# peterWon/D-LIOM

Hardware: NVIDIA H100
Metric: scans/sec (64-beam, 10 Hz) per GPU; pose RMSE vs reference CPU (higher is better)
Workload: dtype f32 (indices, scores) + f64 (pre-integration, least squares)

## Files before the change

d-liom_b200/csrc/dl_voxel.cu:

```cuda
#include <algorithm>
#include <cstdlib>

#include "dl_internal.cuh"

namespace dl {
namespace {

constexpr uint32_t kEmpty = 0xFFFFFFFFu;
constexpr int kBlock = 256;

__device__ __forceinline__ uint32_t hash_cell(const Int3& c) {
  uint32_t h = (uint32_t)c.x * 73856093u ^ (uint32_t)c.y * 19349663u ^ (uint32_t)c.z * 83492791u;
  h ^= h >> 15;
  h *= 0x2c1b3c6du;
  h ^= h >> 12;
  return h;
}
__device__ __forceinline__ Int3 row_cell(const float* __restrict__ pts, int stride, uint32_t row, float res) {
  const float* p = pts + (size_t)row * stride;
  return cell_index(Vec3f{p[0], p[1], p[2]}, res);
}

template <typename RowOf>
__device__ __forceinline__ uint32_t table_insert(uint32_t* table, uint32_t mask, const float* pts, int stride,
// ... 16 lines not shown
                                                              float res, uint32_t* table, int64_t table_cap,
                                                              uint32_t* slot) {
  const int b = blockIdx.y;
  const int n = counts[b];
  const float* pts = points + (size_t)b * cap * stride;
  uint32_t* tab = table + (size_t)b * table_cap;
  const uint32_t mask = (uint32_t)table_cap - 1;
  for (int i = blockIdx.x * kBlock + threadIdx.x; i < n; i += gridDim.x * kBlock) {
    const Int3 c = row_cell(pts, stride, i, res);
    slot[(size_t)b * cap + i] = table_insert(tab, mask, pts, stride, res, c, (uint32_t)i, [](uint32_t id) { return id; });
  }
}

__device__ __forceinline__ int block_exclusive_scan(int value, int* total) {
  __shared__ int warp_sums[kBlock / 32];
  const int lane = threadIdx.x & 31, warp = threadIdx.x >> 5;
  int inc = value;
#pragma unroll
  for (int d = 1; d < 32; d <<= 1) {
    const int o = __shfl_up_sync(0xffffffffu, inc, d);
    if (lane >= d) inc += o;
  }
  __syncthreads();
  if (lane == 31) warp_sums[warp] = inc;
  __syncthreads();
  int base = 0, sum = 0;
#pragma unroll
  for (int w = 0; w < kBlock / 32; ++w) {
    const int s = warp_sums[w];
    if (w < warp) base += s;
    sum += s;
  }
  *total = sum;
  return base + inc - value;
}

__global__ void __launch_bounds__(kBlock) voxel_count_kernel(const int32_t* __restrict__ counts, int64_t cap,
                                                             const uint32_t* __restrict__ table, int64_t table_cap,
                                                             const uint32_t* __restrict__ slot, int32_t* block_counts,
                                                             int tiles) {
  const int b = blockIdx.y;
  const int n = counts[b];
  const int i = blockIdx.x * kBlock + threadIdx.x;
  int flag = 0;
  if (i < n) flag = __ldcg(table + (size_t)b * table_cap + slot[(size_t)b * cap + i]) == (uint32_t)i;
  int total;
  block_exclusive_scan(flag, &total);
  if (threadIdx.x == 0) block_counts[(size_t)b * tiles + blockIdx.x] = total;
}

__global__ void __launch_bounds__(kBlock) voxel_scatter_kernel(const int32_t* __restrict__ counts, int64_t cap,
                                                               const uint32_t* __restrict__ table, int64_t table_cap,
                                                               const uint32_t* __restrict__ slot,
                                                               const int32_t* __restrict__ block_counts, int tiles,
                                                               int32_t* keep, int32_t* keep_counts) {
  const int b = blockIdx.y;
  const int n = counts[b];
  __shared__ int tile_base;
  int partial = 0;
  for (int t = threadIdx.x; t < (int)blockIdx.x; t += kBlock) partial += block_counts[(size_t)b * tiles + t];
  int total;
  block_exclusive_scan(partial, &total);
  if (threadIdx.x == 0) tile_base = total;
  __syncthreads();
  const int i = blockIdx.x * kBlock + threadIdx.x;
  int flag = 0;
  if (i < n) flag = __ldcg(table + (size_t)b * table_cap + slot[(size_t)b * cap + i]) == (uint32_t)i;
  const int off = block_exclusive_scan(flag, &total);
  if (flag) keep[(size_t)b * cap + tile_base + off] = i;
  if (blockIdx.x == gridDim.x - 1 && threadIdx.x == 0) keep_counts[b] = tile_base + total;
}

__global__ void voxel_indices_kernel(const float* __restrict__ points, int stride, int64_t n, float res,
                                     int32_t* __restrict__ out) {
  const int64_t i = (int64_t)blockIdx.x * blockDim.x + threadIdx.x;
  if (i >= n) return;
  const float* p = points + (size_t)i * stride;
  const Int3 c = cell_index(Vec3f{p[0], p[1], p[2]}, make_divider(res));
  out[3 * i] = c.x;
  out[3 * i + 1] = c.y;
  out[3 * i + 2] = c.z;
}

constexpr int kAdaptiveBlock = 1024;
constexpr int kAdaptiveWarps = kAdaptiveBlock / 32;

__device__ __forceinline__ int block_sum_1024(int v) {
  __shared__ int ws[32];
  __shared__ int result;
  const int lane = threadIdx.x & 31, warp = threadIdx.x >> 5;
#pragma unroll
  for (int d = 16; d > 0; d >>= 1) v += __shfl_xor_sync(0xffffffffu, v, d);
  __syncthreads();
  if (lane == 0) ws[warp] = v;
  __syncthreads();
  if (warp == 0) {
    int s = lane < kAdaptiveWarps ? ws[lane] : 0;
#pragma unroll
    for (int d = 16; d > 0; d >>= 1) s += __shfl_xor_sync(0xffffffffu, s, d);
    if (lane == 0) result = s;
  }
  __syncthreads();
  return result;
}

__device__ __forceinline__ int warp_bases_1024(int warp_value, int* total) {
  __shared__ int ws[kAdaptiveWarps], wb[kAdaptiveWarps + 1];
  const int lane = threadIdx.x & 31, warp = threadIdx.x >> 5;
  __syncthreads();
  if (lane == 0) ws[warp] = warp_value;
  __syncthreads();
  if (warp == 0) {
    const int v = ws[lane];
    int inc = v;
#pragma unroll
    for (int d = 1; d < 32; d <<= 1) {
      const int o = __shfl_up_sync(0xffffffffu, inc, d);
      if (lane >= d) inc += o;
    }
    wb[lane] = inc - v;
    if (lane == 31) wb[kAdaptiveWarps] = inc;
  }
  __syncthreads();
  *total = wb[kAdaptiveWarps];
  return wb[warp];
}

template <typename Pred, typename Emit>
__device__ __forceinline__ int block_compact_1024(int n, Pred pred, Emit emit) {
  const int lane = threadIdx.x & 31, warp = threadIdx.x >> 5;
  const int chunk = ((n + kAdaptiveBlock - 1) / kAdaptiveBlock) * 32;
  const int begin = warp * chunk, end = min(n, begin + chunk);
  int count = 0;
  for (int base = begin; base < end; base += 128) {
    bool f[4];
#pragma unroll
    for (int u = 0; u < 4; ++u) {
      const int i = base + 32 * u + lane;
      f[u] = i < end && pred(i);
    }
#pragma unroll
    for (int u = 0; u < 4; ++u) count += __popc(__ballot_sync(0xffffffffu, f[u]));
  }
  int total;
  int pos = warp_bases_1024(count, &total);
  for (int base = begin; base < end; base += 128) {
    bool f[4];
#pragma unroll
    for (int u = 0; u < 4; ++u) {
      const int i = base + 32 * u + lane;
      f[u] = i < end && pred(i);
    }
#pragma unroll
    for (int u = 0; u < 4; ++u) {
      const unsigned ballot = __ballot_sync(0xffffffffu, f[u]);
      if (f[u]) emit(pos + __popc(ballot & ((1u << lane) - 1)), base + 32 * u + lane);
      pos += __popc(ballot);
    }
  }
  __syncthreads();
  return total;
}

template <typename RunPass>
__device__ __forceinline__ bool adaptive_search(const AdaptiveParams& opt, RunPass run_pass, float* result_edge) {
  *result_edge = opt.max_length;
  int result_count = run_pass(opt.max_length);
  if (result_count < 0) return false;
  if ((float)result_count >= opt.min_num_points) return true;
  for (float high_length = opt.max_length; high_length > 1e-2f * opt.max_length; high_length /= 2.f) {
    float low_length = high_length / 2.f;
    result_count = run_pass(low_length);
    if (result_count < 0) return false;
    *result_edge = low_length;
    if ((float)result_count >= opt.min_num_points) {
      while ((high_length - low_length) / low_length > 1e-1f) {
        const float mid_length = (low_length + high_length) / 2.f;
        const int candidate = run_pass(mid_length);
        if (candidate < 0) return false;
        if ((float)candidate >= opt.min_num_points) {
          low_length = mid_length;
          *result_edge = mid_length;
        } else {
          high_length = mid_length;
        }
      }
      return true;
    }
  }
  return true;
}

constexpr int kFastPoints = 8;
constexpr int kFastSlots = 4096;
constexpr int kFastExtra = 14336;
constexpr int kFastCapacity = kFastPoints * 1024 + kFastExtra;
static_assert(kFastCapacity / 1024 <= 32, "the compaction keeps one round count per lane");
constexpr unsigned long long kEmptyKey = 0xFFFFFFFFFFFFFFFFull;

struct FastTable {
  unsigned long long keys[kFastSlots];
  uint32_t mins[kFastSlots];
  float extra[kFastExtra * 3];
};

__device__ __forceinline__ bool pack_cell(const Int3& c, unsigned long long* key) {
  const int lim = 1 << 20;
  if (c.x < -lim || c.x >= lim - 1 || c.y < -lim || c.y >= lim - 1 || c.z < -lim || c.z >= lim - 1) return false;
  *key = ((unsigned long long)(c.x + lim) << 42) | ((unsigned long long)(c.y + lim) << 21) | (unsigned long long)(c.z + lim);
  return true;
}
__device__ __forceinline__ uint32_t hash_key(unsigned long long k) {
  k ^= k >> 33;
  k *= 0xff51afd7ed558ccdull;
  k ^= k >> 29;
  return (uint32_t)k;
}

__device__ __forceinline__ int fast_insert(FastTable& tab, bool have, float x, float y, float z, int j,
                                           const CellDivider& edge, int* fail_flag) {
  const int lane = threadIdx.x & 31;
  unsigned long long key = kEmptyKey - 1 - lane;
  bool ok = true;
  if (have) ok = pack_cell(cell_index(Vec3f{x, y, z}, edge), &key);
  if (!ok) *fail_flag = 1;
  const unsigned peers = __match_any_sync(0xffffffffu, key);
  int claimed = 0;
  if (have && ok && (__ffs(peers) - 1) == lane) {
    uint32_t h = hash_key(key) & (kFastSlots - 1);
    int probes = 0;
    for (;;) {
      const unsigned long long prev = atomicCAS(&tab.keys[h], kEmptyKey, key);
      if (prev == kEmptyKey) claimed = 1;
      if (prev == kEmptyKey || prev == key) {
        atomicMin(&tab.mins[h], (uint32_t)j);
        break;
      }
      h = (h + 1) & (kFastSlots - 1);
      if (++probes >= kFastSlots) {
        *fail_flag = 1;
        break;
      }
    }
  }
  return claimed;
}

__device__ __forceinline__ int fast_pass(FastTable& tab, const float (&px)[kFastPoints], const float (&py)[kFastPoints],
                                         const float (&pz)[kFastPoints], int m, float edge_length, int* fail_flag) {
  const CellDivider edge = make_divider(edge_length);
  for (int i = threadIdx.x; i < kFastSlots; i += kAdaptiveBlock) {
    tab.keys[i] = kEmptyKey;
    tab.mins[i] = 0xFFFFFFFFu;
  }
  __syncthreads();
  int claims = 0;
#pragma unroll
  for (int k = 0; k < kFastPoints; ++k) {
    if (k * kAdaptiveBlock >= m) break;
    const int j = k * kAdaptiveBlock + threadIdx.x;
    claims += fast_insert(tab, j < m, px[k], py[k], pz[k], j, edge, fail_flag);
  }
  for (int base = kFastPoints * kAdaptiveBlock; base < m; base += kAdaptiveBlock) {
    const int j = base + threadIdx.x;
    const float* e = tab.extra + (size_t)(j - kFastPoints * kAdaptiveBlock) * 3;
    const bool have = j < m;
    claims += fast_insert(tab, have, have ? e[0] : 0.f, have ? e[1] : 0.f, have ? e[2] : 0.f, j, edge, fail_flag);
  }
  const int total = block_sum_1024(claims);
  return *fail_flag ? -1 : total;
}

constexpr int kByteCells = (int)((sizeof(unsigned long long) + sizeof(uint32_t)) * kFastSlots);
struct CloudBox {
  float lo[3], hi[3];
};
__device__ __forceinline__ int byte_map_pass(FastTable& tab, const CloudBox& box, const float (&px)[kFastPoints],
                                             const float (&py)[kFastPoints], const float (&pz)[kFastPoints], int m, float edge_length,
                                             int* fail_flag) {
  const CellDivider edge = make_divider(edge_length);
  const Int3 lo = cell_index(Vec3f{box.lo[0], box.lo[1], box.lo[2]}, edge), hi = cell_index(Vec3f{box.hi[0], box.hi[1], box.hi[2]}, edge);
  const long long nx = (long long)hi.x - lo.x + 1, ny = (long long)hi.y - lo.y + 1, nz = (long long)hi.z - lo.z + 1;
  if (nx <= 0 || ny <= 0 || nz <= 0 || nx > kByteCells || ny > kByteCells || nz > kByteCells || nx * ny * nz > kByteCells) return -2;
  const int inx = (int)nx, iny = (int)ny, cells = (int)(nx * ny * nz);
  uint8_t* map = reinterpret_cast<uint8_t*>(&tab);
  uint4* map4 = reinterpret_cast<uint4*>(&tab);
  const int words16 = (cells + 15) >> 4;
  for (int i = threadIdx.x; i < words16; i += kAdaptiveBlock) map4[i] = make_uint4(0u, 0u, 0u, 0u);
  __syncthreads();
  auto mark = [&](float x, float y, float z) {
    const Int3 c = cell_index(Vec3f{x, y, z}, edge);
    const unsigned idx = (unsigned)(((c.z - lo.z) * iny + (c.y - lo.y)) * inx + (c.x - lo.x));
    if (idx < (unsigned)cells) map[idx] = 1;
    else *fail_flag = 1;
  };
#pragma unroll
  for (int k = 0; k < kFastPoints; ++k) {
    if (k * kAdaptiveBlock >= m) break;
    if (k * kAdaptiveBlock + (int)threadIdx.x < m) mark(px[k], py[k], pz[k]);
  }
  for (int j = kFastPoints * kAdaptiveBlock + threadIdx.x; j < m; j += kAdaptiveBlock) {
    const float* e = tab.extra + (size_t)(j - kFastPoints * kAdaptiveBlock) * 3;
    mark(e[0], e[1], e[2]);
  }
  __syncthreads();
  int local = 0;
  for (int i = threadIdx.x; i < words16; i += kAdaptiveBlock) {
    const uint4 v = map4[i];
    local += __popc(v.x) + __popc(v.y) + __popc(v.z) + __popc(v.w);
  }
  const int total = block_sum_1024(local);
  return *fail_flag ? -1 : total;
}

__device__ __forceinline__ bool fast_survives(const FastTable& tab, float x, float y, float z, float edge, int j) {
  unsigned long long key;
  pack_cell(cell_index(Vec3f{x, y, z}, make_divider(edge)), &key);
  uint32_t h = hash_key(key) & (kFastSlots - 1);
  while (tab.keys[h] != key) h = (h + 1) & (kFastSlots - 1);
  return tab.mins[h] == (uint32_t)j;
}

__global__ void __launch_bounds__(kAdaptiveBlock) adaptive_voxel_kernel(
    const float* __restrict__ points, int stride, int64_t cap, const int32_t* __restrict__ counts,
    const AdaptiveParams* __restrict__ filters, int num_filters, uint32_t* table, int64_t table_cap,
    uint32_t* scratch , int32_t* keep, int32_t* keep_counts,
    float* passes, int32_t* num_passes, int32_t* cropped_counts, const int32_t* __restrict__ need) {
  extern __shared__ __align__(16) unsigned char smem_raw[];
  FastTable& fast = *reinterpret_cast<FastTable*>(smem_raw);
  __shared__ int fail_flag;
  const int pair = blockIdx.x;
  if (need && need[4 * pair] == 0) return;
  const int b = pair / num_filters;
  const AdaptiveParams opt = filters[pair % num_filters];
  const int n = counts[b];
  const float* pts = points + (size_t)b * cap * stride;
  uint32_t* tab = table + (size_t)pair * table_cap;
  uint32_t* rows = scratch + (size_t)pair * 2 * cap;
  uint32_t* slot = rows + cap;
  int32_t* out = keep + (size_t)pair * cap;
  float* pass_log = passes + (size_t)pair * 32;
  int npass = 0;
  if (threadIdx.x == 0) fail_flag = 0;

  const int m = block_compact_1024(
      n,
      [&](int i) {
        const float* p = pts + (size_t)i * stride;
        return norm3(Vec3f{p[0], p[1], p[2]}) <= opt.max_range;
      },
      [&](int pos, int i) { rows[pos] = (uint32_t)i; });
  if (threadIdx.x == 0 && cropped_counts) cropped_counts[pair] = m;

  if ((float)m <= opt.min_num_points) {
    for (int j = threadIdx.x; j < m; j += kAdaptiveBlock) out[j] = (int32_t)rows[j];
    if (threadIdx.x == 0) {
      keep_counts[pair] = m;
      num_passes[pair] = 0;
    }
    return;
  }
  auto log_pass = [&](float edge) {
    if (threadIdx.x == 0 && npass < 32) pass_log[npass] = edge;
    ++npass;
  };

  if (m <= kFastCapacity) {
    float px[kFastPoints], py[kFastPoints], pz[kFastPoints];
#pragma unroll
    for (int k = 0; k < kFastPoints; ++k) {
      const int j = k * kAdaptiveBlock + threadIdx.x;
      px[k] = py[k] = pz[k] = 0.f;
      if (j < m) {
        const float* p = pts + (size_t)rows[j] * stride;
        px[k] = p[0]; py[k] = p[1]; pz[k] = p[2];
      }
    }
    for (int j = kFastPoints * kAdaptiveBlock + threadIdx.x; j < m; j += kAdaptiveBlock) {
      const float* p = pts + (size_t)rows[j] * stride;
      float* e = fast.extra + (size_t)(j - kFastPoints * kAdaptiveBlock) * 3;
      e[0] = p[0]; e[1] = p[1]; e[2] = p[2];
    }
    __shared__ CloudBox box;
    __shared__ float box_warp[6][kAdaptiveWarps];
    {
      float lo3[3] = {3.4e38f, 3.4e38f, 3.4e38f}, hi3[3] = {-3.4e38f, -3.4e38f, -3.4e38f};
      auto grow = [&](float x, float y, float z) {
        lo3[0] = fminf(lo3[0], x); lo3[1] = fminf(lo3[1], y); lo3[2] = fminf(lo3[2], z);
        hi3[0] = fmaxf(hi3[0], x); hi3[1] = fmaxf(hi3[1], y); hi3[2] = fmaxf(hi3[2], z);
      };
#pragma unroll
      for (int k = 0; k < kFastPoints; ++k)
        if (k * kAdaptiveBlock + (int)threadIdx.x < m) grow(px[k], py[k], pz[k]);
      for (int j = kFastPoints * kAdaptiveBlock + threadIdx.x; j < m; j += kAdaptiveBlock) {
        const float* p = pts + (size_t)rows[j] * stride;
        grow(p[0], p[1], p[2]);
      }
#pragma unroll
      for (int a3 = 0; a3 < 3; ++a3)
#pragma unroll
        for (int d = 16; d > 0; d >>= 1) {
          lo3[a3] = fminf(lo3[a3], __shfl_xor_sync(0xffffffffu, lo3[a3], d));
          hi3[a3] = fmaxf(hi3[a3], __shfl_xor_sync(0xffffffffu, hi3[a3], d));
        }
      const int lane = threadIdx.x & 31, warp = threadIdx.x >> 5;
      if (lane == 0)
#pragma unroll
        for (int a3 = 0; a3 < 3; ++a3) {
          box_warp[a3][warp] = lo3[a3];
          box_warp[3 + a3][warp] = hi3[a3];
        }
      __syncthreads();
      if (threadIdx.x < 6) {
        float v = box_warp[threadIdx.x][0];
        for (int w = 1; w < kAdaptiveWarps; ++w) v = threadIdx.x < 3 ? fminf(v, box_warp[threadIdx.x][w]) : fmaxf(v, box_warp[threadIdx.x][w]);
        if (threadIdx.x < 3) box.lo[threadIdx.x] = v; else box.hi[threadIdx.x - 3] = v;
      }
    }
    __syncthreads();
    float last_edge = -1.f, result_edge = 0.f;
    const bool ok = adaptive_search(
        opt,
        [&](float edge) {
          log_pass(edge);
          const int count = byte_map_pass(fast, box, px, py, pz, m, edge, &fail_flag);
          if (count != -2) {
            last_edge = -1.f;
            return count;
          }
          last_edge = edge;
          return fast_pass(fast, px, py, pz, m, edge, &fail_flag);
        },
        &result_edge);
    bool done = ok;
    if (ok && last_edge != result_edge) done = fast_pass(fast, px, py, pz, m, result_edge, &fail_flag) >= 0;
    if (done) {
      __shared__ int seq[32 * kAdaptiveWarps];
      const int lane = threadIdx.x & 31, warp = threadIdx.x >> 5;
      const int rounds = (m + kAdaptiveBlock - 1) / kAdaptiveBlock;
      uint32_t flags = 0;
      int my_round_count = 0;
      auto test_round = [&](int k, float x, float y, float z) {
        const int j = k * kAdaptiveBlock + threadIdx.x;
        const bool f = j < m && fast_survives(fast, x, y, z, result_edge, j);
        const unsigned ballot = __ballot_sync(0xffffffffu, f);
        if (f) flags |= 1u << k;
        if (lane == k) my_round_count = __popc(ballot);
      };
#pragma unroll
      for (int k = 0; k < kFastPoints; ++k) {
        if (k >= rounds) break;
        test_round(k, px[k], py[k], pz[k]);
      }
      for (int k = kFastPoints; k < rounds; ++k) {
        const float* e = fast.extra + (size_t)(min(k * kAdaptiveBlock + (int)threadIdx.x, m - 1) - kFastPoints * kAdaptiveBlock) * 3;
        test_round(k, e[0], e[1], e[2]);
      }
      if (lane < rounds) seq[lane * kAdaptiveWarps + warp] = my_round_count;
      __syncthreads();
      const int entries = rounds * kAdaptiveWarps;
      const int v = (int)threadIdx.x < entries ? seq[threadIdx.x] : 0;
      int inc = v;
#pragma unroll
      for (int d = 1; d < 32; d <<= 1) {
        const int o = __shfl_up_sync(0xffffffffu, inc, d);
        if (lane >= d) inc += o;
      }
      int kept;
      const int wbase = warp_bases_1024(__shfl_sync(0xffffffffu, inc, 31), &kept);
      if ((int)threadIdx.x < entries) seq[threadIdx.x] = wbase + inc - v;
      __syncthreads();
      for (int k = 0; k < rounds; ++k) {
        const bool f = (flags >> k) & 1u;
        const unsigned ballot = __ballot_sync(0xffffffffu, f);
        if (f) out[seq[k * kAdaptiveWarps + warp] + __popc(ballot & ((1u << lane) - 1))] = (int32_t)rows[k * kAdaptiveBlock + threadIdx.x];
      }
      if (threadIdx.x == 0) {
        keep_counts[pair] = kept;
        num_passes[pair] = npass;
      }
      return;
    }
    npass = 0;
    __syncthreads();
  }

  uint32_t eff_cap = 64;
  while (eff_cap < 2u * (uint32_t)m) eff_cap <<= 1;
  if (eff_cap > (uint32_t)table_cap) eff_cap = (uint32_t)table_cap;
  const uint32_t mask = eff_cap - 1;
  float last_edge = -1.f;
  auto run_pass = [&](float edge) -> int {
    for (uint32_t i = threadIdx.x; i < eff_cap; i += kAdaptiveBlock) tab[i] = kEmpty;
    __syncthreads();
    for (int j = threadIdx.x; j < m; j += kAdaptiveBlock) {
      const Int3 c = row_cell(pts, stride, rows[j], edge);
      slot[j] = table_insert(tab, mask, pts, stride, edge, c, (uint32_t)j, [&](uint32_t id) { return rows[id]; });
    }
    __syncthreads();
    int local = 0;
    for (int j = threadIdx.x; j < m; j += kAdaptiveBlock) local += __ldcg(tab + slot[j]) == (uint32_t)j;
    last_edge = edge;
    return block_sum_1024(local);
  };
  float result_edge = 0.f;
  adaptive_search(
      opt,
      [&](float edge) {
        log_pass(edge);
        return run_pass(edge);
      },
      &result_edge);
  if (last_edge != result_edge) run_pass(result_edge);
  const int kept = block_compact_1024(
      m, [&](int j) { return __ldcg(tab + slot[j]) == (uint32_t)j; }, [&](int pos, int j) { out[pos] = (int32_t)rows[j]; });
  if (threadIdx.x == 0) {
    keep_counts[pair] = kept;
    num_passes[pair] = npass;
  }
}

constexpr int kEdgeSlots = 8192;
struct EdgeMeta {
  int32_t cropped, voxels, fail, need;
};
__device__ __forceinline__ unsigned long long* edge_keys(uint32_t* table, int64_t table_cap, int pair) {
  return reinterpret_cast<unsigned long long*>(table + (size_t)pair * table_cap);
}
__device__ __forceinline__ uint32_t* edge_mins(uint32_t* table, int64_t table_cap, int pair) {
  return table + (size_t)pair * table_cap + 2 * kEdgeSlots;
}

__global__ void __launch_bounds__(kBlock) adaptive_first_insert_kernel(const float* __restrict__ points, int stride, int64_t cap,
                                                                       const int32_t* __restrict__ counts,
                                                                       const AdaptiveParams* __restrict__ filters, int num_filters,
                                                                       uint32_t* table, int64_t table_cap, uint8_t* win, EdgeMeta* meta) {
  const int pair = blockIdx.y, b = pair / num_filters;
  const AdaptiveParams opt = filters[pair % num_filters];
  const int n = counts[b];
  const float* pts = points + (size_t)b * cap * stride;
  unsigned long long* keys = edge_keys(table, table_cap, pair);
  uint32_t* mins = edge_mins(table, table_cap, pair);
  uint8_t* w = win + (size_t)pair * cap;
  const CellDivider edge = make_divider(opt.max_length);
  int cropped = 0;
  for (int base = blockIdx.x * kBlock; base < n; base += gridDim.x * kBlock) {
    const int i = base + threadIdx.x;
    bool in = false;
    Vec3f p{0.f, 0.f, 0.f};
    if (i < n) {
      const float* q = pts + (size_t)i * stride;
      p = {q[0], q[1], q[2]};
      in = norm3(p) <= opt.max_range;
      w[i] = in ? 2 : 0;
    }
    cropped += in;
    if (in) {
      unsigned long long key;
      if (!pack_cell(cell_index(p, edge), &key)) {
        meta[pair].fail = 1;
      } else {
        uint32_t h = hash_key(key) & (kEdgeSlots - 1);
        int probes = 0;
        for (;;) {
          const unsigned long long prev = atomicCAS(keys + h, kEmptyKey, key);
          if (prev == kEmptyKey || prev == key) {
            atomicMin(mins + h, (uint32_t)i);
            break;
          }
          h = (h + 1) & (kEdgeSlots - 1);
          if (++probes >= kEdgeSlots) {
            meta[pair].fail = 1;
            break;
          }
        }
      }
    }
  }
#pragma unroll
  for (int d = 16; d > 0; d >>= 1) cropped += __shfl_xor_sync(0xffffffffu, cropped, d);
  if ((threadIdx.x & 31) == 0 && cropped) atomicAdd(&meta[pair].cropped, cropped);
}

__global__ void __launch_bounds__(kBlock) adaptive_first_mark_kernel(uint32_t* table, int64_t table_cap, int64_t cap, uint8_t* win,
                                                                     EdgeMeta* meta) {
  const int pair = blockIdx.y;
  const uint32_t* mins = edge_mins(table, table_cap, pair);
  const int h = blockIdx.x * kBlock + threadIdx.x;
  const uint32_t m = __ldcg(mins + h);
  const bool used = m != kEmpty;
  if (used) win[(size_t)pair * cap + m] = 3;
  const int c = __syncthreads_count(used);
  if (threadIdx.x == 0 && c) atomicAdd(&meta[pair].voxels, c);
}

__device__ __forceinline__ int edge_mode(const EdgeMeta& m, const AdaptiveParams& opt) {
  if (m.fail) return 0;
// ... 76 lines not shown

}

int launch_voxel_filter(dl_context* ctx, const float* points, int stride, int64_t cap, const int32_t* counts, int batch,
                        float resolution, uint32_t* table, int64_t table_cap, uint32_t* slot, int32_t* keep,
                        int32_t* keep_counts, int32_t* block_counts) {
  if (batch <= 0 || cap <= 0) return DL_OK;
  DL_CUDA(ctx, cudaMemsetAsync(table, 0xFF, (size_t)batch * table_cap * sizeof(uint32_t), ctx->stream));
  const int tiles = (int)((cap + kBlock - 1) / kBlock);
  const dim3 grid(tiles, batch);
  voxel_insert_kernel<<<grid, kBlock, 0, ctx->stream>>>(points, stride, cap, counts, resolution, table, table_cap, slot);
  DL_LAUNCH_CHECK(ctx, "voxel_insert_kernel");
  voxel_count_kernel<<<grid, kBlock, 0, ctx->stream>>>(counts, cap, table, table_cap, slot, block_counts, tiles);
  DL_LAUNCH_CHECK(ctx, "voxel_count_kernel");
  voxel_scatter_kernel<<<grid, kBlock, 0, ctx->stream>>>(counts, cap, table, table_cap, slot, block_counts, tiles, keep,
                                                         keep_counts);
  DL_LAUNCH_CHECK(ctx, "voxel_scatter_kernel");
  return DL_OK;
}

int launch_voxel_indices(dl_context* ctx, const float* points, int stride, int64_t n, float resolution, int32_t* out) {
  if (n <= 0) return DL_OK;
  voxel_indices_kernel<<<(unsigned)((n + 255) / 256), 256, 0, ctx->stream>>>(points, stride, n, resolution, out);
  DL_LAUNCH_CHECK(ctx, "voxel_indices_kernel");
  return DL_OK;
}

size_t adaptive_first_pass_bytes(int pairs, int64_t cap) {
  const size_t tiles = (size_t)((cap + kBlock - 1) / kBlock);
  return (((size_t)pairs * cap + 255) & ~size_t(255)) + (size_t)pairs * tiles * 4 + (size_t)pairs * sizeof(EdgeMeta) + 256;
}

int launch_adaptive_voxel_filter(dl_context* ctx, const float* points, int stride, int64_t cap, const int32_t* counts,
                                 int batch, const AdaptiveParams* filters_dev, int num_filters, uint32_t* table,
                                 int64_t table_cap, uint32_t* scratch, int32_t* keep, int32_t* keep_counts,
                                 float* passes, int32_t* num_passes, int32_t* cropped_counts, void* first_pass_scratch) {
  if (batch <= 0 || num_filters <= 0) return DL_OK;
  const int pairs = batch * num_filters;
  const int tiles = (int)((cap + kBlock - 1) / kBlock);
  bool first_pass = first_pass_scratch && (size_t)table_cap * 4 >= (size_t)kEdgeSlots * 12;
  if (first_pass && !ctx->h_adaptive_stats) {
    if (cudaMallocHost((void**)&ctx->h_adaptive_stats, 2 * sizeof(int32_t)) != cudaSuccess ||
        cudaMalloc((void**)&ctx->d_adaptive_stats, 2 * sizeof(int32_t)) != cudaSuccess) {
      cudaGetLastError();
      ctx->h_adaptive_stats = nullptr;
    } else {
      ctx->h_adaptive_stats[0] = ctx->h_adaptive_stats[1] = 0;
    }
  }
  int32_t* stats = nullptr;
  if (first_pass && ctx->h_adaptive_stats) {
    const int32_t fell = ctx->h_adaptive_stats[0], probed = ctx->h_adaptive_stats[1];
    const bool probe = (ctx->adaptive_calls++ % 16) == 0;
    if (!probe && probed > 0 && 2 * fell > probed) first_pass = false;
    if (first_pass && probe) stats = ctx->d_adaptive_stats;
  }
  const int32_t* need = nullptr;
  if (first_pass) {
    uint8_t* win = reinterpret_cast<uint8_t*>(first_pass_scratch);
    int32_t* tile_counts = reinterpret_cast<int32_t*>(win + (((size_t)pairs * cap + 255) & ~size_t(255)));
    EdgeMeta* meta = reinterpret_cast<EdgeMeta*>(tile_counts + (size_t)pairs * tiles);
    DL_CUDA(ctx, cudaMemset2DAsync(table, (size_t)table_cap * 4, 0xFF, (size_t)kEdgeSlots * 12, (size_t)pairs, ctx->stream));
    DL_CUDA(ctx, cudaMemsetAsync(meta, 0, sizeof(EdgeMeta) * pairs, ctx->stream));
    if (stats) DL_CUDA(ctx, cudaMemsetAsync(stats, 0, 2 * sizeof(int32_t), ctx->stream));
    const int insert_tiles = std::min(tiles, 96);
    adaptive_first_insert_kernel<<<dim3(insert_tiles, pairs), kBlock, 0, ctx->stream>>>(points, stride, cap, counts, filters_dev,
                                                                                         num_filters, table, table_cap, win, meta);
    DL_LAUNCH_CHECK(ctx, "adaptive_first_insert_kernel");
    adaptive_first_mark_kernel<<<dim3(kEdgeSlots / kBlock, pairs), kBlock, 0, ctx->stream>>>(table, table_cap, cap, win, meta);
    DL_LAUNCH_CHECK(ctx, "adaptive_first_mark_kernel");
    adaptive_first_count_kernel<<<dim3(tiles, pairs), kBlock, 0, ctx->stream>>>(counts, filters_dev, num_filters, cap, win, meta,
                                                                                 tile_counts, tiles);
    DL_LAUNCH_CHECK(ctx, "adaptive_first_count_kernel");
    adaptive_first_prefix_kernel<<<pairs, kBlock, 0, ctx->stream>>>(counts, filters_dev, num_filters, meta, tile_counts, tiles,
                                                                    keep_counts, passes, num_passes, cropped_counts, stats);
    DL_LAUNCH_CHECK(ctx, "adaptive_first_prefix_kernel");
    if (stats)
      DL_CUDA(ctx, cudaMemcpyAsync(ctx->h_adaptive_stats, stats, 2 * sizeof(int32_t), cudaMemcpyDeviceToHost, ctx->stream));
    adaptive_first_scatter_kernel<<<dim3(tiles, pairs), kBlock, 0, ctx->stream>>>(counts, filters_dev, num_filters, cap, win, meta,
                                                                                   tile_counts, tiles, keep);
    DL_LAUNCH_CHECK(ctx, "adaptive_first_scatter_kernel");
    need = &meta->need;
  }
  DL_CUDA(ctx, cudaFuncSetAttribute(adaptive_voxel_kernel, cudaFuncAttributeMaxDynamicSharedMemorySize, (int)sizeof(FastTable)));
  adaptive_voxel_kernel<<<pairs, kAdaptiveBlock, sizeof(FastTable), ctx->stream>>>(
      points, stride, cap, counts, filters_dev, num_filters, table, table_cap, scratch, keep, keep_counts, passes,
      num_passes, cropped_counts, need);
  DL_LAUNCH_CHECK(ctx, "adaptive_voxel_kernel");
  return DL_OK;
}

}
```

Baseline: 110,100.

## Restructure adaptive voxel search into multi-edge count sweeps with speculative edges

Rewrites the adaptive voxel kernel: instead of caching points in registers/shared memory and running one hash or byte-map pass per candidate edge, it replays the search against a table of known counts. It evaluates up to three speculative edges per sweep over global points using packed occupancy bitmaps in a 32KB static shared union. The final survivors go through a small shared hash, and output order comes from a rank sort. The block shrinks from 1024 to 512 threads with two blocks per SM, and a fast rounding-based cell index is added with an exact fallback. It risks more global reads per sweep, a quadratic rank sort when many voxels survive, and falling back to the global-table path when more than 2048 cells survive or the bounding box overflows the map.

```diff
diff --git a/d-liom_b200/csrc/dl_voxel.cu b/d-liom_b200/csrc/dl_voxel.cu
--- a/d-liom_b200/csrc/dl_voxel.cu
+++ b/d-liom_b200/csrc/dl_voxel.cu
@@ -122,11 +122,16 @@
   out[3 * i + 2] = c.z;
 }
 
-constexpr int kAdaptiveBlock = 1024;
-constexpr int kAdaptiveWarps = kAdaptiveBlock / 32;
-
-__device__ __forceinline__ int block_sum_1024(int v) {
-  __shared__ int ws[32];
+constexpr int kSearchBlock = 512;
+constexpr int kSearchWarps = kSearchBlock / 32;
+constexpr int kMapBytes = 32768;
+constexpr int kResultSlots = 2048;
+constexpr int kMaxAhead = 3;
+constexpr int kKnownEdges = 64;
+constexpr unsigned long long kEmptyKey = 0xFFFFFFFFFFFFFFFFull;
+
+__device__ __forceinline__ int block_sum(int v) {
+  __shared__ int ws[kSearchWarps];
   __shared__ int result;
   const int lane = threadIdx.x & 31, warp = threadIdx.x >> 5;
 #pragma unroll
@@ -135,7 +140,7 @@
   if (lane == 0) ws[warp] = v;
   __syncthreads();
   if (warp == 0) {
-    int s = lane < kAdaptiveWarps ? ws[lane] : 0;
+    int s = lane < kSearchWarps ? ws[lane] : 0;
 #pragma unroll
     for (int d = 16; d > 0; d >>= 1) s += __shfl_xor_sync(0xffffffffu, s, d);
     if (lane == 0) result = s;
@@ -144,32 +149,32 @@
   return result;
 }
 
-__device__ __forceinline__ int warp_bases_1024(int warp_value, int* total) {
-  __shared__ int ws[kAdaptiveWarps], wb[kAdaptiveWarps + 1];
+__device__ __forceinline__ int warp_bases(int warp_value, int* total) {
+  __shared__ int ws[kSearchWarps], wb[kSearchWarps + 1];
   const int lane = threadIdx.x & 31, warp = threadIdx.x >> 5;
   __syncthreads();
   if (lane == 0) ws[warp] = warp_value;
   __syncthreads();
   if (warp == 0) {
-    const int v = ws[lane];
+    const int v = lane < kSearchWarps ? ws[lane] : 0;
     int inc = v;
 #pragma unroll
     for (int d = 1; d < 32; d <<= 1) {
       const int o = __shfl_up_sync(0xffffffffu, inc, d);
       if (lane >= d) inc += o;
     }
-    wb[lane] = inc - v;
-    if (lane == 31) wb[kAdaptiveWarps] = inc;
-  }
-  __syncthreads();
-  *total = wb[kAdaptiveWarps];
+    if (lane < kSearchWarps) wb[lane] = inc - v;
+    if (lane == 31) wb[kSearchWarps] = inc;
+  }
+  __syncthreads();
+  *total = wb[kSearchWarps];
   return wb[warp];
 }
 
-template <typename Pred, typename Emit>
-__device__ __forceinline__ int block_compact_1024(int n, Pred pred, Emit emit) {
+template <typename Pred>
+__device__ __forceinline__ int warp_chunk_count(int n, Pred pred) {
   const int lane = threadIdx.x & 31, warp = threadIdx.x >> 5;
-  const int chunk = ((n + kAdaptiveBlock - 1) / kAdaptiveBlock) * 32;
+  const int chunk = ((n + kSearchBlock - 1) / kSearchBlock) * 32;
   const int begin = warp * chunk, end = min(n, begin + chunk);
   int count = 0;
   for (int base = begin; base < end; base += 128) {
@@ -182,8 +187,13 @@
 #pragma unroll
     for (int u = 0; u < 4; ++u) count += __popc(__ballot_sync(0xffffffffu, f[u]));
   }
-  int total;
-  int pos = warp_bases_1024(count, &total);
+  return count;
+}
+template <typename Pred, typename Emit>
+__device__ __forceinline__ void warp_chunk_emit(int n, int pos, Pred pred, Emit emit) {
+  const int lane = threadIdx.x & 31, warp = threadIdx.x >> 5;
+  const int chunk = ((n + kSearchBlock - 1) / kSearchBlock) * 32;
+  const int begin = warp * chunk, end = min(n, begin + chunk);
   for (int base = begin; base < end; base += 128) {
     bool f[4];
 #pragma unroll
@@ -199,6 +209,12 @@
     }
   }
   __syncthreads();
+}
+template <typename Pred, typename Emit>
+__device__ __forceinline__ int block_compact(int n, Pred pred, Emit emit) {
+  int total;
+  const int pos = warp_bases(warp_chunk_count(n, pred), &total);
+  warp_chunk_emit(n, pos, pred, emit);
   return total;
 }
 
@@ -231,19 +247,6 @@
   return true;
 }
 
-constexpr int kFastPoints = 8;
-constexpr int kFastSlots = 4096;
-constexpr int kFastExtra = 14336;
-constexpr int kFastCapacity = kFastPoints * 1024 + kFastExtra;
-static_assert(kFastCapacity / 1024 <= 32, "the compaction keeps one round count per lane");
-constexpr unsigned long long kEmptyKey = 0xFFFFFFFFFFFFFFFFull;
-
-struct FastTable {
-  unsigned long long keys[kFastSlots];
-  uint32_t mins[kFastSlots];
-  float extra[kFastExtra * 3];
-};
-
 __device__ __forceinline__ bool pack_cell(const Int3& c, unsigned long long* key) {
   const int lim = 1 << 20;
   if (c.x < -lim || c.x >= lim - 1 || c.y < -lim || c.y >= lim - 1 || c.z < -lim || c.z >= lim - 1) return false;
@@ -257,293 +260,342 @@
   return (uint32_t)k;
 }
 
-__device__ __forceinline__ int fast_insert(FastTable& tab, bool have, float x, float y, float z, int j,
-                                           const CellDivider& edge, int* fail_flag) {
+union SearchShared {
+  uint4 maps[kMapBytes / 16];
+  struct {
+    unsigned long long keys[kResultSlots];
+    uint32_t mins[kResultSlots];
+    uint32_t rows[kResultSlots];
+  } result;
+};
+struct EdgeBox {
+  CellDivider div;
+  int lo[3], nx, ny, cells, map0;
+};
+struct SearchState {
+  float lo[3], hi[3];
+  float box_warp[6][kSearchWarps];
+  int num_set, words;
+  EdgeBox set[kMaxAhead];
+  int set_count[kMaxAhead];
+  int num_known;
+  float known_edge[kKnownEdges];
+  int known_count[kKnownEdges];
+  int fail, survivors;
+};
+
+__device__ __forceinline__ int find_edge(const float* edges, int num, float edge) {
+  for (int k = 0; k < num; ++k)
+    if (__float_as_uint(edges[k]) == __float_as_uint(edge)) return k;
+  return -1;
+}
+
+__device__ bool place_edge(SearchState& st, float edge) {
+  if (find_edge(st.known_edge, st.num_known, edge) >= 0) return true;
+  for (int k = 0; k < st.num_set; ++k)
+    if (__float_as_uint(st.set[k].div.resolution) == __float_as_uint(edge)) return true;
+  if (st.num_set == kMaxAhead || st.num_known + st.num_set == kKnownEdges) return false;
+  const CellDivider div = make_divider(edge);
+  const Int3 lo = cell_index(Vec3f{st.lo[0], st.lo[1], st.lo[2]}, div), hi = cell_index(Vec3f{st.hi[0], st.hi[1], st.hi[2]}, div);
+  const long long nx = (long long)hi.x - lo.x + 1, ny = (long long)hi.y - lo.y + 1, nz = (long long)hi.z - lo.z + 1;
+  const long long budget = 16LL * (kMapBytes / 16 - st.words);
+  if (nx <= 0 || ny <= 0 || nz <= 0 || nx > budget || ny > budget || nz > budget || nx * ny * nz > budget) return false;
+  EdgeBox& b = st.set[st.num_set++];
+  b.div = div;
+  b.lo[0] = lo.x; b.lo[1] = lo.y; b.lo[2] = lo.z;
+  b.nx = (int)nx; b.ny = (int)ny; b.cells = (int)(nx * ny * nz);
+  b.map0 = st.words;
+  st.words += (b.cells + 15) >> 4;
+  return true;
+}
+
+__device__ __forceinline__ bool cell_index_fast(const Vec3f& p, const CellDivider& d, Int3* c) {
+  const float v[3] = {p.x, p.y, p.z};
+  int k[3];
+  bool ok = true;
+#pragma unroll
+  for (int a = 0; a < 3; ++a) {
+    const float q = v[a] * d.inverse;
+    const float aq = fabsf(q);
+    const float t = aq + 12582912.f;
+    const float dist = fabsf(aq - (t - 12582912.f));
+    ok = ok && aq < 4194304.f && 0.5f - dist > aq * 4.8e-7f + 1e-30f;
+    const int r = __float_as_int(t) - 0x4B400000;
+    k[a] = q < 0.f ? -r : r;
+  }
+  *c = Int3{k[0], k[1], k[2]};
+  return ok;
+}
+
+__device__ void count_sweep(SearchShared& sm, SearchState& st, const float* __restrict__ pts, int stride, int n, float max_range) {
+  for (int i = threadIdx.x; i < st.words; i += kSearchBlock) sm.maps[i] = make_uint4(0u, 0u, 0u, 0u);
+  if (threadIdx.x < kMaxAhead) st.set_count[threadIdx.x] = 0;
+  __syncthreads();
+  const int num_set = st.num_set;
+  constexpr int kBatch = 3;
+  for (int base = 0; base < n; base += kBatch * kSearchBlock) {
+    Vec3f v[kBatch];
+    bool in[kBatch];
+#pragma unroll
+    for (int u = 0; u < kBatch; ++u) {
+      const int i = base + u * kSearchBlock + threadIdx.x;
+      in[u] = false;
+      v[u] = Vec3f{0.f, 0.f, 0.f};
+      if (i < n) {
+        const float* p = pts + (size_t)i * stride;
+        v[u] = Vec3f{p[0], p[1], p[2]};
+        in[u] = norm3(v[u]) <= max_range;
+      }
+    }
+    for (int k = 0; k < num_set; ++k) {
+      const EdgeBox b = st.set[k];
+      unsigned idx[kBatch];
+#pragma unroll
+      for (int u = 0; u < kBatch; ++u) {
+        Int3 c;
+        if (!cell_index_fast(v[u], b.div, &c) && in[u]) c = cell_index(v[u], b.div);
+        idx[u] = (unsigned)(((c.z - b.lo[2]) * b.ny + (c.y - b.lo[1])) * b.nx + (c.x - b.lo[0]));
+      }
+      uint8_t* map = reinterpret_cast<uint8_t*>(sm.maps + b.map0);
+#pragma unroll
+      for (int u = 0; u < kBatch; ++u) {
+        if (!in[u]) continue;
+        if (idx[u] < (unsigned)b.cells) map[idx[u]] = 1;
+        else st.fail = 1;
+      }
+    }
+  }
+  __syncthreads();
+  for (int k = 0; k < num_set; ++k) {
+    const EdgeBox& b = st.set[k];
+    int local = 0;
+    for (int i = threadIdx.x; i < (b.cells + 15) >> 4; i += kSearchBlock) {
+      const uint4 v = sm.maps[b.map0 + i];
+      local += __popc(v.x) + __popc(v.y) + __popc(v.z) + __popc(v.w);
+    }
+#pragma unroll
+    for (int d = 16; d > 0; d >>= 1) local += __shfl_xor_sync(0xffffffffu, local, d);
+    if ((threadIdx.x & 31) == 0 && local) atomicAdd(&st.set_count[k], local);
+  }
+  __syncthreads();
+  if (threadIdx.x == 0) {
+    for (int k = 0; k < num_set; ++k) {
+      st.known_edge[st.num_known] = st.set[k].div.resolution;
+      st.known_count[st.num_known++] = st.set_count[k];
+    }
+  }
+  __syncthreads();
+}
+
+__device__ void result_sweep(SearchShared& sm, SearchState& st, const float* __restrict__ pts, int stride, int n, float max_range,
+                             float edge) {
+  for (int i = threadIdx.x; i < kResultSlots; i += kSearchBlock) {
+    sm.result.keys[i] = kEmptyKey;
+    sm.result.mins[i] = kEmpty;
+  }
+  if (threadIdx.x == 0) st.survivors = 0;
+  __syncthreads();
+  const CellDivider div = make_divider(edge);
   const int lane = threadIdx.x & 31;
-  unsigned long long key = kEmptyKey - 1 - lane;
-  bool ok = true;
-  if (have) ok = pack_cell(cell_index(Vec3f{x, y, z}, edge), &key);
-  if (!ok) *fail_flag = 1;
-  const unsigned peers = __match_any_sync(0xffffffffu, key);
-  int claimed = 0;
-  if (have && ok && (__ffs(peers) - 1) == lane) {
-    uint32_t h = hash_key(key) & (kFastSlots - 1);
-    int probes = 0;
-    for (;;) {
-      const unsigned long long prev = atomicCAS(&tab.keys[h], kEmptyKey, key);
-      if (prev == kEmptyKey) claimed = 1;
-      if (prev == kEmptyKey || prev == key) {
-        atomicMin(&tab.mins[h], (uint32_t)j);
-        break;
-      }
-      h = (h + 1) & (kFastSlots - 1);
-      if (++probes >= kFastSlots) {
-        *fail_flag = 1;
-        break;
-      }
-    }
-  }
-  return claimed;
-}
-
-__device__ __forceinline__ int fast_pass(FastTable& tab, const float (&px)[kFastPoints], const float (&py)[kFastPoints],
-                                         const float (&pz)[kFastPoints], int m, float edge_length, int* fail_flag) {
-  const CellDivider edge = make_divider(edge_length);
-  for (int i = threadIdx.x; i < kFastSlots; i += kAdaptiveBlock) {
-    tab.keys[i] = kEmptyKey;
-    tab.mins[i] = 0xFFFFFFFFu;
-  }
-  __syncthreads();
-  int claims = 0;
-#pragma unroll
-  for (int k = 0; k < kFastPoints; ++k) {
-    if (k * kAdaptiveBlock >= m) break;
-    const int j = k * kAdaptiveBlock + threadIdx.x;
-    claims += fast_insert(tab, j < m, px[k], py[k], pz[k], j, edge, fail_flag);
-  }
-  for (int base = kFastPoints * kAdaptiveBlock; base < m; base += kAdaptiveBlock) {
-    const int j = base + threadIdx.x;
-    const float* e = tab.extra + (size_t)(j - kFastPoints * kAdaptiveBlock) * 3;
-    const bool have = j < m;
-    claims += fast_insert(tab, have, have ? e[0] : 0.f, have ? e[1] : 0.f, have ? e[2] : 0.f, j, edge, fail_flag);
-  }
-  const int total = block_sum_1024(claims);
-  return *fail_flag ? -1 : total;
-}
-
-constexpr int kByteCells = (int)((sizeof(unsigned long long) + sizeof(uint32_t)) * kFastSlots);
-struct CloudBox {
-  float lo[3], hi[3];
-};
-__device__ __forceinline__ int byte_map_pass(FastTable& tab, const CloudBox& box, const float (&px)[kFastPoints],
-                                             const float (&py)[kFastPoints], const float (&pz)[kFastPoints], int m, float edge_length,
-                                             int* fail_flag) {
-  const CellDivider edge = make_divider(edge_length);
-  const Int3 lo = cell_index(Vec3f{box.lo[0], box.lo[1], box.lo[2]}, edge), hi = cell_index(Vec3f{box.hi[0], box.hi[1], box.hi[2]}, edge);
-  const long long nx = (long long)hi.x - lo.x + 1, ny = (long long)hi.y - lo.y + 1, nz = (long long)hi.z - lo.z + 1;
-  if (nx <= 0 || ny <= 0 || nz <= 0 || nx > kByteCells || ny > kByteCells || nz > kByteCells || nx * ny * nz > kByteCells) return -2;
-  const int inx = (int)nx, iny = (int)ny, cells = (int)(nx * ny * nz);
-  uint8_t* map = reinterpret_cast<uint8_t*>(&tab);
-  uint4* map4 = reinterpret_cast<uint4*>(&tab);
-  const int words16 = (cells + 15) >> 4;
-  for (int i = threadIdx.x; i < words16; i += kAdaptiveBlock) map4[i] = make_uint4(0u, 0u, 0u, 0u);
-  __syncthreads();
-  auto mark = [&](float x, float y, float z) {
-    const Int3 c = cell_index(Vec3f{x, y, z}, edge);
-    const unsigned idx = (unsigned)(((c.z - lo.z) * iny + (c.y - lo.y)) * inx + (c.x - lo.x));
-    if (idx < (unsigned)cells) map[idx] = 1;
-    else *fail_flag = 1;
-  };
-#pragma unroll
-  for (int k = 0; k < kFastPoints; ++k) {
-    if (k * kAdaptiveBlock >= m) break;
-    if (k * kAdaptiveBlock + (int)threadIdx.x < m) mark(px[k], py[k], pz[k]);
-  }
-  for (int j = kFastPoints * kAdaptiveBlock + threadIdx.x; j < m; j += kAdaptiveBlock) {
-    const float* e = tab.extra + (size_t)(j - kFastPoints * kAdaptiveBlock) * 3;
-    mark(e[0], e[1], e[2]);
-  }
-  __syncthreads();
-  int local = 0;
-  for (int i = threadIdx.x; i < words16; i += kAdaptiveBlock) {
-    const uint4 v = map4[i];
-    local += __popc(v.x) + __popc(v.y) + __popc(v.z) + __popc(v.w);
-  }
-  const int total = block_sum_1024(local);
-  return *fail_flag ? -1 : total;
-}
-
-__device__ __forceinline__ bool fast_survives(const FastTable& tab, float x, float y, float z, float edge, int j) {
-  unsigned long long key;
-  pack_cell(cell_index(Vec3f{x, y, z}, make_divider(edge)), &key);
-  uint32_t h = hash_key(key) & (kFastSlots - 1);
-  while (tab.keys[h] != key) h = (h + 1) & (kFastSlots - 1);
-  return tab.mins[h] == (uint32_t)j;
-}
-
-__global__ void __launch_bounds__(kAdaptiveBlock) adaptive_voxel_kernel(
+  constexpr int kBatch = 4;
+  for (int base = 0; base < n; base += kBatch * kSearchBlock) {
+    unsigned long long key[kBatch];
+    bool have[kBatch];
+#pragma unroll
+    for (int u = 0; u < kBatch; ++u) {
+      const int i = base + u * kSearchBlock + threadIdx.x;
+      key[u] = kEmptyKey - 1 - lane;
+      have[u] = false;
+      if (i < n) {
+        const float* p = pts + (size_t)i * stride;
+        const Vec3f v{p[0], p[1], p[2]};
+        if (norm3(v) <= max_range) {
+          Int3 c;
+          if (!cell_index_fast(v, div, &c)) c = cell_index(v, div);
+          have[u] = pack_cell(c, &key[u]);
+          if (!have[u]) st.fail = 1;
+        }
+      }
+    }
+#pragma unroll
+    for (int u = 0; u < kBatch; ++u) {
+      const unsigned peers = __match_any_sync(0xffffffffu, key[u]);
+      if (have[u] && (__ffs(peers) - 1) == lane) {
+        uint32_t h = hash_key(key[u]) & (kResultSlots - 1);
+        for (int probes = 0;;) {
+          const unsigned long long prev = atomicCAS(&sm.result.keys[h], kEmptyKey, key[u]);
+          if (prev == kEmptyKey || prev == key[u]) {
+            atomicMin(&sm.result.mins[h], (uint32_t)(base + u * kSearchBlock + threadIdx.x));
+            break;
+          }
+          h = (h + 1) & (kResultSlots - 1);
+          if (++probes >= kResultSlots) {
+            st.fail = 1;
+            break;
+          }
+        }
+      }
+    }
+  }
+  __syncthreads();
+}
+
+__global__ void __launch_bounds__(kSearchBlock, 2) adaptive_voxel_kernel(
     const float* __restrict__ points, int stride, int64_t cap, const int32_t* __restrict__ counts,
     const AdaptiveParams* __restrict__ filters, int num_filters, uint32_t* table, int64_t table_cap,
     uint32_t* scratch , int32_t* keep, int32_t* keep_counts,
     float* passes, int32_t* num_passes, int32_t* cropped_counts, const int32_t* __restrict__ need) {
-  extern __shared__ __align__(16) unsigned char smem_raw[];
-  FastTable& fast = *reinterpret_cast<FastTable*>(smem_raw);
-  __shared__ int fail_flag;
+  __shared__ SearchShared sm;
+  __shared__ SearchState st;
   const int pair = blockIdx.x;
   if (need && need[4 * pair] == 0) return;
   const int b = pair / num_filters;
   const AdaptiveParams opt = filters[pair % num_filters];
   const int n = counts[b];
   const float* pts = points + (size_t)b * cap * stride;
-  uint32_t* tab = table + (size_t)pair * table_cap;
-  uint32_t* rows = scratch + (size_t)pair * 2 * cap;
-  uint32_t* slot = rows + cap;
   int32_t* out = keep + (size_t)pair * cap;
   float* pass_log = passes + (size_t)pair * 32;
+  const int lane = threadIdx.x & 31, warp = threadIdx.x >> 5;
+  auto in_range = [&](int i) {
+    const float* p = pts + (size_t)i * stride;
+    return norm3(Vec3f{p[0], p[1], p[2]}) <= opt.max_range;
+  };
+
+  {
+    float lo3[3] = {3.4e38f, 3.4e38f, 3.4e38f}, hi3[3] = {-3.4e38f, -3.4e38f, -3.4e38f};
+    const int count = warp_chunk_count(n, [&](int i) {
+      const float* p = pts + (size_t)i * stride;
+      const float v[3] = {p[0], p[1], p[2]};
+      if (!(norm3(Vec3f{v[0], v[1], v[2]}) <= opt.max_range)) return false;
+#pragma unroll
+      for (int a = 0; a < 3; ++a) {
+        lo3[a] = fminf(lo3[a], v[a]);
+        hi3[a] = fmaxf(hi3[a], v[a]);
+      }
+      return true;
+    });
+#pragma unroll
+    for (int a = 0; a < 3; ++a)
+#pragma unroll
+      for (int d = 16; d > 0; d >>= 1) {
+        lo3[a] = fminf(lo3[a], __shfl_xor_sync(0xffffffffu, lo3[a], d));
+        hi3[a] = fmaxf(hi3[a], __shfl_xor_sync(0xffffffffu, hi3[a], d));
+      }
+    if (lane == 0)
+#pragma unroll
+      for (int a = 0; a < 3; ++a) {
+        st.box_warp[a][warp] = lo3[a];
+        st.box_warp[3 + a][warp] = hi3[a];
+      }
+    if (threadIdx.x == 0) {
+      st.fail = 0;
+      st.num_known = 0;
+    }
+    int m;
+    const int pos = warp_bases(count, &m);
+    if (threadIdx.x < 6) {
+      float v = st.box_warp[threadIdx.x][0];
+      for (int w = 1; w < kSearchWarps; ++w) v = threadIdx.x < 3 ? fminf(v, st.box_warp[threadIdx.x][w]) : fmaxf(v, st.box_warp[threadIdx.x][w]);
+      if (threadIdx.x < 3) st.lo[threadIdx.x] = v;
+      else st.hi[threadIdx.x - 3] = v;
+    }
+    if (threadIdx.x == 0 && cropped_counts) cropped_counts[pair] = m;
+    if ((float)m <= opt.min_num_points) {
+      warp_chunk_emit(n, pos, in_range, [&](int pos, int i) { out[pos] = i; });
+      if (threadIdx.x == 0) {
+        keep_counts[pair] = m;
+        num_passes[pair] = 0;
+      }
+      return;
+    }
+  }
   int npass = 0;
-  if (threadIdx.x == 0) fail_flag = 0;
-
-  const int m = block_compact_1024(
-      n,
-      [&](int i) {
-        const float* p = pts + (size_t)i * stride;
-        return norm3(Vec3f{p[0], p[1], p[2]}) <= opt.max_range;
-      },
-      [&](int pos, int i) { rows[pos] = (uint32_t)i; });
-  if (threadIdx.x == 0 && cropped_counts) cropped_counts[pair] = m;
-
-  if ((float)m <= opt.min_num_points) {
-    for (int j = threadIdx.x; j < m; j += kAdaptiveBlock) out[j] = (int32_t)rows[j];
-    if (threadIdx.x == 0) {
-      keep_counts[pair] = m;
-      num_passes[pair] = 0;
-    }
-    return;
-  }
   auto log_pass = [&](float edge) {
     if (threadIdx.x == 0 && npass < 32) pass_log[npass] = edge;
     ++npass;
   };
 
-  if (m <= kFastCapacity) {
-    float px[kFastPoints], py[kFastPoints], pz[kFastPoints];
-#pragma unroll
-    for (int k = 0; k < kFastPoints; ++k) {
-      const int j = k * kAdaptiveBlock + threadIdx.x;
-      px[k] = py[k] = pz[k] = 0.f;
-      if (j < m) {
-        const float* p = pts + (size_t)rows[j] * stride;
-        px[k] = p[0]; py[k] = p[1]; pz[k] = p[2];
-      }
-    }
-    for (int j = kFastPoints * kAdaptiveBlock + threadIdx.x; j < m; j += kAdaptiveBlock) {
-      const float* p = pts + (size_t)rows[j] * stride;
-      float* e = fast.extra + (size_t)(j - kFastPoints * kAdaptiveBlock) * 3;
-      e[0] = p[0]; e[1] = p[1]; e[2] = p[2];
-    }
-    __shared__ CloudBox box;
-    __shared__ float box_warp[6][kAdaptiveWarps];
-    {
-      float lo3[3] = {3.4e38f, 3.4e38f, 3.4e38f}, hi3[3] = {-3.4e38f, -3.4e38f, -3.4e38f};
-      auto grow = [&](float x, float y, float z) {
-        lo3[0] = fminf(lo3[0], x); lo3[1] = fminf(lo3[1], y); lo3[2] = fminf(lo3[2], z);
-        hi3[0] = fmaxf(hi3[0], x); hi3[1] = fmaxf(hi3[1], y); hi3[2] = fmaxf(hi3[2], z);
-      };
-#pragma unroll
-      for (int k = 0; k < kFastPoints; ++k)
-        if (k * kAdaptiveBlock + (int)threadIdx.x < m) grow(px[k], py[k], pz[k]);
-      for (int j = kFastPoints * kAdaptiveBlock + threadIdx.x; j < m; j += kAdaptiveBlock) {
-        const float* p = pts + (size_t)rows[j] * stride;
-        grow(p[0], p[1], p[2]);
-      }
-#pragma unroll
-      for (int a3 = 0; a3 < 3; ++a3)
-#pragma unroll
-        for (int d = 16; d > 0; d >>= 1) {
-          lo3[a3] = fminf(lo3[a3], __shfl_xor_sync(0xffffffffu, lo3[a3], d));
-          hi3[a3] = fmaxf(hi3[a3], __shfl_xor_sync(0xffffffffu, hi3[a3], d));
-        }
-      const int lane = threadIdx.x & 31, warp = threadIdx.x >> 5;
-      if (lane == 0)
-#pragma unroll
-        for (int a3 = 0; a3 < 3; ++a3) {
-          box_warp[a3][warp] = lo3[a3];
-          box_warp[3 + a3][warp] = hi3[a3];
-        }
-      __syncthreads();
-      if (threadIdx.x < 6) {
-        float v = box_warp[threadIdx.x][0];
-        for (int w = 1; w < kAdaptiveWarps; ++w) v = threadIdx.x < 3 ? fminf(v, box_warp[threadIdx.x][w]) : fmaxf(v, box_warp[threadIdx.x][w]);
-        if (threadIdx.x < 3) box.lo[threadIdx.x] = v; else box.hi[threadIdx.x - 3] = v;
-      }
-    }
+  float result_edge = 0.f;
+  for (;;) {
     __syncthreads();
-    float last_edge = -1.f, result_edge = 0.f;
-    const bool ok = adaptive_search(
+    if (st.fail) break;
+    npass = 0;
+    bool bisecting = false, missed = false;
+    float missing = 0.f;
+    adaptive_search(
         opt,
-        [&](float edge) {
+        [&](float edge) -> int {
+          const int k = find_edge(st.known_edge, st.num_known, edge);
+          if (k < 0) {
+            missed = true;
+            missing = edge;
+            return -1;
+          }
           log_pass(edge);
-          const int count = byte_map_pass(fast, box, px, py, pz, m, edge, &fail_flag);
-          if (count != -2) {
-            last_edge = -1.f;
-            return count;
-          }
-          last_edge = edge;
-          return fast_pass(fast, px, py, pz, m, edge, &fail_flag);
+          const int count = st.known_count[k];
+          if ((float)count >= opt.min_num_points) bisecting = true;
+          return count;
         },
         &result_edge);
-    bool done = ok;
-    if (ok && last_edge != result_edge) done = fast_pass(fast, px, py, pz, m, result_edge, &fail_flag) >= 0;
-    if (done) {
-      __shared__ int seq[32 * kAdaptiveWarps];
-      const int lane = threadIdx.x & 31, warp = threadIdx.x >> 5;
-      const int rounds = (m + kAdaptiveBlock - 1) / kAdaptiveBlock;
-      uint32_t flags = 0;
-      int my_round_count = 0;
-      auto test_round = [&](int k, float x, float y, float z) {
-        const int j = k * kAdaptiveBlock + threadIdx.x;
-        const bool f = j < m && fast_survives(fast, x, y, z, result_edge, j);
-        const unsigned ballot = __ballot_sync(0xffffffffu, f);
-        if (f) flags |= 1u << k;
-        if (lane == k) my_round_count = __popc(ballot);
-      };
-#pragma unroll
-      for (int k = 0; k < kFastPoints; ++k) {
-        if (k >= rounds) break;
-        test_round(k, px[k], py[k], pz[k]);
-      }
-      for (int k = kFastPoints; k < rounds; ++k) {
-        const float* e = fast.extra + (size_t)(min(k * kAdaptiveBlock + (int)threadIdx.x, m - 1) - kFastPoints * kAdaptiveBlock) * 3;
-        test_round(k, e[0], e[1], e[2]);
-      }
-      if (lane < rounds) seq[lane * kAdaptiveWarps + warp] = my_round_count;
-      __syncthreads();
-      const int entries = rounds * kAdaptiveWarps;
-      const int v = (int)threadIdx.x < entries ? seq[threadIdx.x] : 0;
-      int inc = v;
-#pragma unroll
-      for (int d = 1; d < 32; d <<= 1) {
-        const int o = __shfl_up_sync(0xffffffffu, inc, d);
-        if (lane >= d) inc += o;
-      }
-      int kept;
-      const int wbase = warp_bases_1024(__shfl_sync(0xffffffffu, inc, 31), &kept);
-      if ((int)threadIdx.x < entries) seq[threadIdx.x] = wbase + inc - v;
-      __syncthreads();
-      for (int k = 0; k < rounds; ++k) {
-        const bool f = (flags >> k) & 1u;
-        const unsigned ballot = __ballot_sync(0xffffffffu, f);
-        if (f) out[seq[k * kAdaptiveWarps + warp] + __popc(ballot & ((1u << lane) - 1))] = (int32_t)rows[k * kAdaptiveBlock + threadIdx.x];
-      }
-      if (threadIdx.x == 0) {
-        keep_counts[pair] = kept;
-        num_passes[pair] = npass;
-      }
-      return;
-    }
-    npass = 0;
+    if (!missed) break;
     __syncthreads();
-  }
-
+    if (threadIdx.x == 0) {
+      st.num_set = st.words = 0;
+      if (!place_edge(st, missing)) {
+        st.fail = 1;
+      } else if (!bisecting) {
+        const float low = missing / 2.f;
+        if (place_edge(st, low)) place_edge(st, (low + missing) / 2.f);
+      }
+    }
+    __syncthreads();
+    if (st.fail) break;
+    count_sweep(sm, st, pts, stride, n, opt.max_range);
+  }
+  if (!st.fail) result_sweep(sm, st, pts, stride, n, opt.max_range, result_edge);
+  if (!st.fail) {
+    for (int s = threadIdx.x; s < kResultSlots; s += kSearchBlock) {
+      const uint32_t r = sm.result.mins[s];
+      if (r != kEmpty) sm.result.rows[atomicAdd(&st.survivors, 1)] = r;
+    }
+    __syncthreads();
+    const int kept = st.survivors;
+    for (int a = threadIdx.x; a < kept; a += kSearchBlock) {
+      const uint32_t r = sm.result.rows[a];
+      int rank = 0;
+      for (int c = 0; c < kept; ++c) rank += sm.result.rows[c] < r;
+      out[rank] = (int32_t)r;
+    }
+    if (threadIdx.x == 0) {
+      keep_counts[pair] = kept;
+      num_passes[pair] = npass;
+    }
+    return;
+  }
+
+  uint32_t* tab = table + (size_t)pair * table_cap;
+  uint32_t* rows = scratch + (size_t)pair * 2 * cap;
+  uint32_t* slot = rows + cap;
+  const int m = block_compact(n, in_range, [&](int pos, int i) { rows[pos] = (uint32_t)i; });
+  npass = 0;
   uint32_t eff_cap = 64;
   while (eff_cap < 2u * (uint32_t)m) eff_cap <<= 1;
   if (eff_cap > (uint32_t)table_cap) eff_cap = (uint32_t)table_cap;
   const uint32_t mask = eff_cap - 1;
   float last_edge = -1.f;
   auto run_pass = [&](float edge) -> int {
-    for (uint32_t i = threadIdx.x; i < eff_cap; i += kAdaptiveBlock) tab[i] = kEmpty;
+    for (uint32_t i = threadIdx.x; i < eff_cap; i += kSearchBlock) tab[i] = kEmpty;
     __syncthreads();
-    for (int j = threadIdx.x; j < m; j += kAdaptiveBlock) {
+    for (int j = threadIdx.x; j < m; j += kSearchBlock) {
       const Int3 c = row_cell(pts, stride, rows[j], edge);
       slot[j] = table_insert(tab, mask, pts, stride, edge, c, (uint32_t)j, [&](uint32_t id) { return rows[id]; });
     }
     __syncthreads();
     int local = 0;
-    for (int j = threadIdx.x; j < m; j += kAdaptiveBlock) local += __ldcg(tab + slot[j]) == (uint32_t)j;
+    for (int j = threadIdx.x; j < m; j += kSearchBlock) local += __ldcg(tab + slot[j]) == (uint32_t)j;
     last_edge = edge;
-    return block_sum_1024(local);
+    return block_sum(local);
   };
-  float result_edge = 0.f;
   adaptive_search(
       opt,
       [&](float edge) {
@@ -552,7 +604,7 @@
       },
       &result_edge);
   if (last_edge != result_edge) run_pass(result_edge);
-  const int kept = block_compact_1024(
+  const int kept = block_compact(
       m, [&](int j) { return __ldcg(tab + slot[j]) == (uint32_t)j; }, [&](int pos, int j) { out[pos] = (int32_t)rows[j]; });
   if (threadIdx.x == 0) {
     keep_counts[pair] = kept;
@@ -795,8 +847,7 @@
     DL_LAUNCH_CHECK(ctx, "adaptive_first_scatter_kernel");
     need = &meta->need;
   }
-  DL_CUDA(ctx, cudaFuncSetAttribute(adaptive_voxel_kernel, cudaFuncAttributeMaxDynamicSharedMemorySize, (int)sizeof(FastTable)));
-  adaptive_voxel_kernel<<<pairs, kAdaptiveBlock, sizeof(FastTable), ctx->stream>>>(
+  adaptive_voxel_kernel<<<pairs, kSearchBlock, 0, ctx->stream>>>(
       points, stride, cap, counts, filters_dev, num_filters, table, table_cap, scratch, keep, keep_counts, passes,
       num_passes, cropped_counts, need);
   DL_LAUNCH_CHECK(ctx, "adaptive_voxel_kernel");
```

New measurement: 116,800 (median of 6 runs). +6.1%, better.
